# ChenJiahao031008/EAO-Fusion

Hardware: AMD Instinct MI355X
Metric: ORB kpts/s (640x480, 1k feat) + local-BA residuals/s (20 KF x 3k pts) (higher is better)
Workload: dtype u8; 1 GPU; ORBextractor FAST+rBRIEF, 640x480, 8-level pyramid, nFeatures 1000, batch=64 synthetic frames per GPU (BASELINE configs[1]); parallelism=frames sharded per GPU, no data-path collective

## Files before the change

### eao_fusion_amd/csrc/orb_host.hip

```cpp
#include "orb_internal.h"

using namespace eao::orb;

namespace eao {
namespace orb {

eao_status build_geometry(eao_orb* h, int W, int H) {
    const eao_orb_cfg& c = h->cfg;
    Geom& g = h->geom;
    std::memset(&g, 0, sizeof(g));
    g.nlevels = c.nlevels; g.W = W; g.H = H;
    g.iniTh = c.ini_th_fast; g.minTh = c.min_th_fast;
    for (int i = 0; i < 16; i++) g.umax[i] = h->umax[i];
    h->cells.clear();
    int off = 0, kpBase = 0, candBase = 0, tileBase = 0, maxCell = 0, scanCap = 0, maxList = 0, maxSw = 0, maxSh = 0;
    for (int l = 0; l < c.nlevels; l++) {
        LevelGeom& L = g.L[l];
        const float s = h->invScale[l];
        L.w = cv_round((float)W * s);
        L.h = cv_round((float)H * s);
        EAO_REQUIRE(L.w < 4096 && L.h < 4096, "level %d is %dx%d: coordinates are packed in 12 bits", l, L.w, L.h);
        const int maxBX = L.w - kEdge + 3, maxBY = L.h - kEdge + 3;
        const float width = (float)(maxBX - kMinBorder), height = (float)(maxBY - kMinBorder);
        const int nCols = (int)(width / (float)refc::FAST_CELL), nRows = (int)(height / (float)refc::FAST_CELL);
// ... 348 lines not shown
    const int nl = cfg->nlevels;
    const double scaleFactor = cfg->scale_factor;
    h->scale.resize(nl); h->sigma2.resize(nl); h->invScale.resize(nl); h->invSigma2.resize(nl); h->quota.resize(nl);
    h->scale[0] = 1.0f; h->sigma2[0] = 1.0f;
    for (int i = 1; i < nl; i++) {
        h->scale[i] = (float)(h->scale[i - 1] * scaleFactor);
        h->sigma2[i] = h->scale[i] * h->scale[i];
    }
    for (int i = 0; i < nl; i++) {
        h->invScale[i] = 1.0f / h->scale[i];
        h->invSigma2[i] = 1.0f / h->sigma2[i];
    }
    const float factor = (float)(1.0f / scaleFactor);
    float desired = cfg->nfeatures * (1 - factor) / (1 - (float)std::pow((double)factor, (double)nl));
    int sum = 0;
    for (int l = 0; l < nl - 1; l++) {
        h->quota[l] = cv_round(desired);
        sum += h->quota[l];
        desired *= factor;
    }
    h->quota[nl - 1] = std::max(cfg->nfeatures - sum, 0);
    {
        const int vmax = (int)std::floor(15 * std::sqrt(2.f) / 2 + 1), vmin = (int)std::ceil(15 * std::sqrt(2.f) / 2);
        for (int v = 0; v <= vmax; ++v) h->umax[v] = cv_round(std::sqrt(225.0 - v * v));
        for (int v = 15, v0 = 0; v >= vmin; --v) {
            while (h->umax[v0] == h->umax[v0 + 1]) ++v0;
            h->umax[v] = v0;
            ++v0;
        }
    }
    {
        const int expect[16] = {15, 15, 15, 15, 14, 14, 14, 13, 13, 12, 11, 10, 9, 8, 6, 3};
        for (int i = 0; i < 16; i++)
            if (h->umax[i] != expect[i]) { delete h; eao::set_error("umax table mismatch"); return EAO_ERR_INTERNAL; }
    }
    *out = h;
    return EAO_OK;
}

void eao_orb_destroy(eao_orb* h) {
    if (!h) return;
    for (hipEvent_t e : h->evs) if (e) (void)hipEventDestroy(e);
    if (h->stream) { (void)hipStreamSynchronize(h->stream); (void)hipStreamDestroy(h->stream); }
    for (hipStream_t q : {h->spacer, h->side}) if (q) { (void)hipStreamSynchronize(q); (void)hipStreamDestroy(q); }
    for (hipEvent_t e : {h->evFork, h->evFast0, h->evMid, h->evJoin}) if (e) (void)hipEventDestroy(e);
    if (h->pinOut) (void)hipHostFree(h->pinOut);
    if (h->pinUp) (void)hipHostFree(h->pinUp);
    if (h->pinPyr) (void)hipHostFree(h->pinPyr);
    stream_release(h);
    if (h->evStart) (void)hipEventDestroy(h->evStart);
    if (h->evLast) (void)hipEventDestroy(h->evLast);
    delete h;
}

eao_status eao_orb_tables(const eao_orb* h, float* scale, float* inv_scale, float* sigma2, float* inv_sigma2, int32_t* fpl) {
    EAO_REQUIRE(h, "null handle");
    for (int i = 0; i < h->cfg.nlevels; i++) {
        if (scale) scale[i] = h->scale[i];
        if (inv_scale) inv_scale[i] = h->invScale[i];
        if (sigma2) sigma2[i] = h->sigma2[i];
        if (inv_sigma2) inv_sigma2[i] = h->invSigma2[i];
        if (fpl) fpl[i] = h->quota[i];
    }
    return EAO_OK;
}

eao_status eao_orb_max_keypoints(eao_orb* h, int32_t width, int32_t height, int32_t* cap) {
    EAO_REQUIRE(h && cap, "null argument");
    eao_status st = ensure(h, width, height, 0);
    if (st) return st;
    *cap = h->geom.totalKpCap;
    return EAO_OK;
}

eao_status eao_orb_extract_batch_device(eao_orb* h, const uint8_t* d_img, int32_t width, int32_t height, int32_t stride,
                                        int64_t frame_stride, int32_t batch, eao_keypoint* d_kps, uint8_t* d_desc, int32_t cap,
                                        int32_t* d_n, void* stream) {
    EAO_REQUIRE(h && d_img && d_kps && d_desc && d_n, "null argument");
    EAO_REQUIRE(width > 0 && height > 0 && stride >= width && batch >= 1, "bad image geometry");
    eao_status st = ensure(h, width, height, batch, (hipStream_t)stream);
    if (st) return st;
    if (cap < h->geom.totalKpCap) {
        eao::set_error("cap %d < eao_orb_max_keypoints %d", cap, h->geom.totalKpCap);
        return EAO_ERR_CAPACITY;
    }
    return enqueue(h, d_img, stride, frame_stride, batch, d_kps, d_desc, cap, d_n, (hipStream_t)stream);
}

eao_status eao_orb_extract_batch(eao_orb* h, const uint8_t* img, int32_t width, int32_t height, int32_t stride, int64_t frame_stride,
                                 int32_t batch, eao_keypoint* kps, uint8_t* desc, int32_t cap, int32_t* n) {
    EAO_REQUIRE(h && n, "null argument");
    if (!img || width <= 0 || height <= 0) {
        for (int f = 0; f < std::max(batch, 0); f++) n[f] = 0;
        return EAO_OK;
    }
    EAO_REQUIRE(kps && desc && stride >= width && batch >= 1, "bad argument");
    eao_status st = ensure(h, width, height, batch);
    if (st) return st;
    const Geom& g = h->geom;
    if (cap < g.totalKpCap) {
        eao::set_error("cap %d < eao_orb_max_keypoints %d", cap, g.totalKpCap);
        return EAO_ERR_CAPACITY;
    }
    const size_t B = batch;
    if ((st = h->d_in.reserve(B * (size_t)g.L[0].pitch * height))) return st;
    if ((st = h->d_kps.reserve(B * (size_t)cap))) return st;
    if ((st = h->d_desc.reserve(B * (size_t)cap * 32))) return st;
    if ((st = h->d_nout.reserve(B))) return st;
    const long long fs0 = (long long)g.L[0].pitch * height;
    if ((st = upload_frames(h, img, width, height, stride, frame_stride, batch))) return st;
    const size_t outBytes = B * sizeof(int) + 64 + B * (size_t)cap * (sizeof(eao_keypoint) + 32);
    if (outBytes <= kPinnedOutMax) {
        if (h->pinOutCap < outBytes) {
            if (h->pinOut) (void)hipHostFree(h->pinOut);
            h->pinOut = nullptr; h->pinOutCap = 0;
            EAO_HIP(hipHostMalloc((void**)&h->pinOut, outBytes, hipHostMallocMapped));
            h->pinOutCap = outBytes;
        }
        unsigned char* dv = nullptr;
        EAO_HIP(hipHostGetDevicePointer((void**)&dv, h->pinOut, 0));
        const size_t offK = (B * sizeof(int) + 63) & ~(size_t)63, offD = offK + B * (size_t)cap * sizeof(eao_keypoint);
        st = enqueue(h, h->d_in.p, g.L[0].pitch, fs0, batch, (eao_keypoint*)(dv + offK), dv + offD, cap, (int*)dv, h->stream);
        if (st) return st;
        EAO_HIP(eao::wait_latency(h->stream));
        h->lastComplete = true;
        const int* hn = (const int*)h->pinOut;
        for (int f = 0; f < batch; f++) {
            const int nf = std::min(std::max(hn[f], 0), cap);
            n[f] = nf;
            std::memcpy(kps + (size_t)f * cap, h->pinOut + offK + (size_t)f * cap * sizeof(eao_keypoint), (size_t)nf * sizeof(eao_keypoint));
            std::memcpy(desc + (size_t)f * cap * 32, h->pinOut + offD + (size_t)f * cap * 32, (size_t)nf * 32);
        }
        return EAO_OK;
    }
    st = enqueue(h, h->d_in.p, g.L[0].pitch, fs0, batch, h->d_kps.p, h->d_desc.p, cap, h->d_nout.p, h->stream);
    if (st) return st;
    EAO_HIP(hipMemcpyAsync(n, h->d_nout.p, B * sizeof(int), hipMemcpyDeviceToHost, h->stream));
    EAO_HIP(hipMemcpyAsync(kps, h->d_kps.p, B * cap * sizeof(eao_keypoint), hipMemcpyDeviceToHost, h->stream));
    EAO_HIP(hipMemcpyAsync(desc, h->d_desc.p, B * (size_t)cap * 32, hipMemcpyDeviceToHost, h->stream));
    EAO_HIP(eao::wait_latency(h->stream));
    h->lastComplete = true;
    return EAO_OK;
}

eao_status eao_orb_extract(eao_orb* h, const uint8_t* img, int32_t width, int32_t height, int32_t stride, eao_keypoint* kps,
                           uint8_t* desc, int32_t cap, int32_t* n) {
    return eao_orb_extract_batch(h, img, width, height, stride, 0, 1, kps, desc, cap, n);
}

eao_status eao_orb_stream_create(eao_orb* h, int32_t width, int32_t height, int32_t batch, int32_t nslots) {
    EAO_REQUIRE(h && width > 0 && height > 0 && batch >= 1 && nslots >= 1 && nslots <= 8, "bad argument (1..8 slots)");
    eao_status st = ensure(h, width, height, batch);
    if (st) return st;
    stream_release(h);
    const Geom& g = h->geom;
    h->sW = width; h->sH = height; h->sB = batch; h->sCap = g.totalKpCap; h->sPitch = g.L[0].pitch;
    const size_t B = batch, cap = h->sCap;
    h->sInBytes = B * (size_t)h->sPitch * height;
    h->sOffK = eao::align256(B * sizeof(int));
    h->sOffD = eao::align256(h->sOffK + B * cap * sizeof(eao_keypoint));
    h->sOutBytes = (h->sOffD + B * cap * 32 + 15) & ~(size_t)15;
    EAO_HIP(eao::create_stream(&h->sUp, eao::StreamClass::Latency));
    EAO_HIP(eao::create_stream(&h->sRun, eao::StreamClass::Latency));
    EAO_HIP(eao::create_stream(&h->sDown, eao::StreamClass::Latency));
    h->slots.resize(nslots);
    for (eao_orb::StreamSlot& sl : h->slots) {
        EAO_HIP(hipHostMalloc((void**)&sl.pinIn, h->sInBytes, hipHostMallocDefault));
        EAO_HIP(hipHostMalloc((void**)&sl.pinOut, h->sOutBytes, hipHostMallocMapped));
        EAO_HIP(hipHostGetDevicePointer((void**)&sl.pinOutDev, sl.pinOut, 0));
        EAO_HIP(hipMalloc((void**)&sl.dIn, h->sInBytes));
        EAO_HIP(hipMalloc((void**)&sl.dOut, h->sOutBytes));
        EAO_HIP(hipEventCreateWithFlags(&sl.evIn, hipEventDisableTiming));
        EAO_HIP(hipEventCreateWithFlags(&sl.evOut, hipEventDisableTiming));
        EAO_HIP(hipEventCreateWithFlags(&sl.evDone, hipEventDisableTiming));
        std::memset(sl.pinOut, 0, h->sOutBytes);
    }
    return EAO_OK;
}

eao_status eao_orb_stream_slot(eao_orb* h, int32_t slot, eao_orb_slot* out) {
    EAO_REQUIRE(h && out && slot >= 0 && slot < (int)h->slots.size(), "no such slot (eao_orb_stream_create first)");
    const eao_orb::StreamSlot& sl = h->slots[slot];
    out->frames = sl.pinIn; out->stride = h->sPitch; out->frame_stride = (int64_t)h->sPitch * h->sH;
    out->n = (int32_t*)sl.pinOut; out->kps = (eao_keypoint*)(sl.pinOut + h->sOffK); out->desc = sl.pinOut + h->sOffD; out->cap = h->sCap;
    return EAO_OK;
}

eao_status eao_orb_stream_wait(eao_orb* h, int32_t slot) {
    EAO_REQUIRE(h && slot >= 0 && slot < (int)h->slots.size(), "no such slot (eao_orb_stream_create first)");
    eao_orb::StreamSlot& sl = h->slots[slot];
    EAO_REQUIRE(sl.submitted, "slot %d was not submitted", slot);
    EAO_HIP(hipEventSynchronize(sl.evOut));
    EAO_HIP(hipGetLastError());
    return EAO_OK;
}

eao_status eao_orb_level(eao_orb* h, int32_t frame, int32_t level, int32_t which, int32_t* w, int32_t* hgt, uint8_t* dst) {
    EAO_REQUIRE(h && h->geomValid && h->lastBatch > 0, "no extraction has run on this handle");
    EAO_REQUIRE(frame >= 0 && frame < h->lastBatch && level >= 0 && level < h->geom.nlevels, "frame/level out of range");
    const LevelGeom& L = h->geom.L[level];
    if (w) *w = L.w;
    if (hgt) *hgt = L.h;
    if (!dst) return EAO_OK;
    const uint8_t* src;
    int pitch;
    if (which == 0 && level == 0) {
        src = h->lastSrc.img0 + (long long)frame * h->lastSrc.fs0;
        pitch = h->lastSrc.pitch0;
    } else {
        src = (which ? h->d_blur.p : h->d_pyr.p) + (long long)frame * h->geom.pyrFrameBytes + L.off;
        pitch = L.pitch;
    }
    eao_status st = wait_last_extraction(h);
    if (st) return st;
    EAO_HIP(hipMemcpy2DAsync(dst, L.w, src, pitch, L.w, L.h, hipMemcpyDeviceToHost, h->stream));
    EAO_HIP(eao::wait_latency(h->stream));
    return EAO_OK;
}

eao_status eao_orb_pyramid(eao_orb* h, int32_t frame, int32_t border, eao_orb_level_view* levels) {
    EAO_REQUIRE(h && levels && h->geomValid && h->lastBatch > 0, "no extraction has run on this handle");
    EAO_REQUIRE(frame >= 0 && frame < h->lastBatch && border >= 0 && border <= 64, "frame / border out of range");
    if (!(h->lastComplete && h->pyrFrame == frame && h->pyrBorder == border)) {
        eao_status st = wait_last_extraction(h);
        if (!st) st = enqueue_pyramid_export(h, frame, border);
        if (st) return st;
        EAO_HIP(eao::wait_latency(h->stream));
        EAO_HIP(hipGetLastError());
    }
    for (int l = 0; l < h->geom.nlevels; l++) levels[l] = h->pyrViews[l];
    return EAO_OK;
}

eao_status eao_orb_set_keep_pyramid(eao_orb* h, int32_t border) {
    EAO_REQUIRE(h && border >= -1 && border <= 64, "border: -1 (off) .. 64");
    h->autoPyrBorder = border;
    return EAO_OK;
}

eao_status eao_orb_extract_ref(eao_orb* h, const uint8_t* img, int32_t width, int32_t height, int32_t stride, const eao_keypoint** kps,
                               const uint8_t** desc, int32_t* n) {
    EAO_REQUIRE(h && kps && desc && n, "null argument");
    *kps = nullptr; *desc = nullptr; *n = 0;
    if (!img || width <= 0 || height <= 0) return EAO_OK;
    EAO_REQUIRE(stride >= width, "bad argument");
    eao_status st = ensure(h, width, height, 1);
    if (st) return st;
    const Geom& g = h->geom;
    const int cap = g.totalKpCap;
    const size_t offK = 64, offD = offK + (size_t)cap * sizeof(eao_keypoint), outBytes = offD + (size_t)cap * 32;
    if (h->pinOutCap < outBytes) {
        if (h->pinOut) (void)hipHostFree(h->pinOut);
        h->pinOut = nullptr; h->pinOutCap = 0;
        EAO_HIP(hipHostMalloc((void**)&h->pinOut, outBytes, hipHostMallocMapped));
        h->pinOutCap = outBytes;
    }
    unsigned char* dv = nullptr;
    EAO_HIP(hipHostGetDevicePointer((void**)&dv, h->pinOut, 0));
    if ((st = h->d_in.reserve((size_t)g.L[0].pitch * height))) return st;
    const long long fs0 = (long long)g.L[0].pitch * height;
    if ((st = upload_frames(h, img, width, height, stride, 0, 1))) return st;
    st = enqueue(h, h->d_in.p, g.L[0].pitch, fs0, 1, (eao_keypoint*)(dv + offK), dv + offD, cap, (int*)dv, h->stream);
    if (st) return st;
    if (h->autoPyrBorder >= 0 && (st = enqueue_pyramid_export(h, 0, h->autoPyrBorder))) return st;
    EAO_HIP(eao::wait_latency(h->stream));
    h->lastComplete = true;
    *n = std::min(std::max(*(const int*)h->pinOut, 0), cap);
    *kps = (const eao_keypoint*)(h->pinOut + offK);
    *desc = h->pinOut + offD;
    return EAO_OK;
}

int32_t eao_orb_lanes(int32_t) { return 1; }

eao_status eao_orb_set_profiling(eao_orb* h, int32_t on) {
    EAO_REQUIRE(h, "null handle");
    h->profiling = on != 0;
    h->evUsed = 0;
    return EAO_OK;
}

eao_status eao_orb_last_timing(eao_orb* h, float ms[6]) {
    EAO_REQUIRE(h && ms && h->evUsed >= kProfEvents, "no profiled call since eao_orb_set_profiling(h, 1)");
    const size_t calls = h->evUsed / kProfEvents;
    EAO_HIP(hipEventSynchronize(h->evs[h->evUsed - kProfEvents + 8]));
    double acc[6] = {0, 0, 0, 0, 0, 0};
    for (size_t c = 0; c < calls; c++) {
        hipEvent_t* ev = &h->evs[c * kProfEvents];
        float t;
        EAO_HIP(hipEventElapsedTime(&t, ev[0], ev[1])); acc[0] += t;
        EAO_HIP(hipEventElapsedTime(&t, ev[9], ev[2])); acc[1] += t;
        EAO_HIP(hipEventElapsedTime(&t, ev[2], ev[3])); acc[2] += t;
        EAO_HIP(hipEventElapsedTime(&t, ev[6], ev[7])); acc[3] += t;
        EAO_HIP(hipEventElapsedTime(&t, ev[4], ev[5])); acc[4] += t;
        EAO_HIP(hipEventElapsedTime(&t, ev[0], ev[8])); acc[5] += t;
    }
    for (int i = 0; i < 6; i++) ms[i] = (float)(acc[i] / calls);
    h->evUsed = 0;
    if (h->d_dbg) {
        long long st[16 * kMaxLevels];
        EAO_HIP(hipMemcpy(st, h->d_dbg, sizeof(st), hipMemcpyDeviceToHost));
        for (int l = 0; l < h->geom.nlevels; l++) {
            const long long* o = st + 16 * l;
            fprintf(stderr, "[eao quadtree stamps] level %d: M %lld S %lld passes %lld | setup %lld | multi-scan %lld hist %lld order %lld growth %lld rank %lld newlist %lld rehome %lld tail %lld | final %lld cycles\n",
                    l, o[10], o[11], o[9], o[0], o[1], o[2], o[3], o[4], o[5], o[6], o[7], 0LL, o[8]);
        }
    }
    return EAO_OK;
}

}
```

### eao_fusion_amd/csrc/orb_internal.h

```cpp
#pragma once

#include <algorithm>
#include <atomic>
#include <cmath>
#include <cstdlib>
#include <cstring>
#include <vector>

#include "common.h"
#include "orb_blur_tables.h"
#include "orb_resize_tables.h"


namespace eao {
namespace orb {

constexpr int kMaxLevels = 16;
constexpr int kEdge = refc::EDGE_THRESHOLD;
constexpr int kMinBorder = kEdge - 3;
constexpr int kTile = 72;
constexpr int kTileStrideWide = 80;
constexpr int kMaxIni = 16;
constexpr size_t kPinnedOutMax = 1 << 20;
constexpr int kFastXcdRun = 0;

struct LevelGeom {
    int w, h, pitch, off;
    int cellBase, nCells;
    int quota;
    int nIni, boxH;
    float hX;
    int listCap;
    int kpBase;
    int candBase, candCap;
    int tileBase, tilesX;
    int mOk, mTileBase;
    int mTilesX, mBlocksY;
    int mXIdx, mYIdx;
    long long nodeOff;
    int scaledPatch;
    float scale;
};

struct Geom {
    int nlevels, W, H;
    int totalCells, cellCap;
    int totalKpCap, totalCandCap, totalTiles;
    int mTotalTiles, mFragOff;
    int pyrFrameBytes;
    int iniTh, minTh;
    int scanCap;
    int qtLdsCand, qtKeysOff;
    int qtNodesGlobal;
    long long qtNodeFrameBytes;
    int fastMaxTested, fastTileBytes, fastLdsBytes, fastStride;
    int umax[16];
    LevelGeom L[kMaxLevels];
};

struct CellDesc {
    short level, x0, y0, sw, sh, offX, offY, pad;
};

struct ImgSrc {
    const uint8_t* img0;
    int pitch0;
    long long fs0;
    uint8_t* pyr;
};

__device__ __forceinline__ const uint8_t* level_ptr(const Geom* g, const ImgSrc& s, int l, int f, int* pitch) {
    if (l == 0) {
        *pitch = s.pitch0;
        return s.img0 + (long long)f * s.fs0;
    }
    *pitch = g->L[l].pitch;
    return s.pyr + (long long)f * g->pyrFrameBytes + g->L[l].off;
}

constexpr int kPyrTW = 128, kPyrTH = 32;
constexpr int kPyrThreads = 256;
struct PyrLevel { int w, h, pitch, off; double invX, invY; int ldsOff, ldsW, ldsH; int coefXOff, coefYOff; };
struct PyrArgs {
    int nlevels, tilesX, tilesY, pyrFrameBytes;
    int coefOff;
    int coefCap;
    PyrLevel L[kMaxLevels];
    const int4* ranges;
    const int2* coefX;
    const int2* coefY;
};

constexpr int kQTSmall = 1024, kQTLarge = 256;
constexpr int kQtNodeInts = 2 + 2 + 2 + 4 + 4 + 5;

constexpr size_t kProfEvents = 10;


__host__ __device__ inline int pyr_src_ofs(int d, double inv, int sn) {
    float fr = (float)(((double)d + 0.5) * inv - 0.5);
    int o = (int)floorf(fr);
    return o < 0 ? 0 : (o > sn - 1 ? sn - 1 : o);
}
__host__ __device__ inline int pyr_first_at_least(int bound, double inv, int sn, int dn) {
    if (bound <= 0) return 0;
    int d = (int)((double)bound / inv);
    d = d < 0 ? 0 : (d > dn ? dn : d);
    while (d > 0 && pyr_src_ofs(d - 1, inv, sn) >= bound) d--;
    while (d < dn && pyr_src_ofs(d, inv, sn) < bound) d++;
    return d;
}

constexpr int kBlurRows = 16;
constexpr int kBlurSegW = 128;
constexpr int kBlurStripsPerWg = 8;
inline int cv_round(double v) { return (int)std::lrint(v); }

}
}

struct eao_orb {
    using Geom = eao::orb::Geom; using CellDesc = eao::orb::CellDesc; using PyrArgs = eao::orb::PyrArgs; using ImgSrc = eao::orb::ImgSrc;
    eao_orb_cfg cfg;
    std::vector<float> scale, invScale, sigma2, invSigma2;
    std::vector<int> quota;
    int umax[16];
    Geom geom;
    bool geomValid = false;
    int batchCap = 0;
    std::vector<CellDesc> cells;
    size_t quadLds = 0;
    eao::DevBuf<int4> d_pyrRanges;
    eao::DevBuf<int2> d_pyrCoef;
    PyrArgs pyr;
    size_t pyrLds = 0;
    bool pyrFused = false;
    hipStream_t stream = nullptr;
    hipStream_t side = nullptr;
    hipStream_t spacer = nullptr;
    bool evLastValid = false;
    hipStream_t lastStream = nullptr;
    hipEvent_t evLast = nullptr;
    bool everyCallEvent = false, evLastRecorded = false;
    hipEvent_t evStart = nullptr, evFork = nullptr, evJoin = nullptr, evFast0 = nullptr, evMid = nullptr;
    eao::DevBuf<Geom> d_geom;
    eao::DevBuf<CellDesc> d_cells;
    eao::DevBuf<uint8_t> d_pyr, d_blur, d_in;
    eao::DevBuf<uint8_t> d_blurTab;
    eao::DevBuf<uint8_t> d_resizeTab;
    eao::orb::ResizeMLevel resizeM[eao::orb::kMaxLevels] = {};
    size_t resizeMRowsOff = 0, resizeMStripsOff = 0;
    eao::DevBuf<unsigned> d_cellcand, d_cand, d_levelkps;
    eao::DevBuf<unsigned short> d_nodeof;
    eao::DevBuf<unsigned char> d_qtnodes;
    eao::DevBuf<int> d_cellcnt, d_levelcnt, d_candcnt, d_nout;
    eao::DevBuf<eao_keypoint> d_kps;
    unsigned char* pinOut = nullptr;
    size_t pinOutCap = 0;
    unsigned char* pinUp = nullptr;
    size_t pinUpCap = 0;
    eao::DevBuf<uint8_t> d_desc;
    eao::DevBuf<float> d_xyr;
    eao::DevBuf<unsigned char> d_stereo;
    unsigned char* pinPyr = nullptr;
    size_t pinPyrCap = 0;
    eao_orb_level_view pyrViews[eao::orb::kMaxLevels] = {};
    int pyrFrame = -1, pyrBorder = -1;
    int autoPyrBorder = -1;
    bool lastComplete = false;
    ImgSrc lastSrc{};
    int lastBatch = 0;
    bool profiling = false;
    long long* d_dbg = nullptr;
    std::vector<hipEvent_t> evs;
    size_t evUsed = 0;
    struct StreamSlot {
        unsigned char* pinIn = nullptr; unsigned char* pinOut = nullptr;
        unsigned char* pinOutDev = nullptr;
        unsigned char* dIn = nullptr; unsigned char* dOut = nullptr;
        hipEvent_t evIn = nullptr, evDone = nullptr, evOut = nullptr;
        int batch = 0;
        bool submitted = false;
    };
    std::vector<StreamSlot> slots;
    hipStream_t sUp = nullptr, sRun = nullptr, sDown = nullptr;
    int sW = 0, sH = 0, sB = 0, sCap = 0, sPitch = 0;
    size_t sInBytes = 0, sOutBytes = 0, sOffK = 0, sOffD = 0;
};

namespace eao {
namespace orb {
constexpr uintptr_t kNoCallerStream = ~(uintptr_t)0;
eao_status ensure(eao_orb* h, int W, int H, int batch, hipStream_t caller = (hipStream_t)kNoCallerStream);
eao_status order_behind_last_call(eao_orb* h, hipStream_t st);
void stream_release(eao_orb* h);
eao_status wait_last_extraction(eao_orb* h);
eao_status upload_frames(eao_orb* h, const uint8_t* img, int width, int height, int stride, long long frame_stride, int batch);
eao_status enqueue(eao_orb* h, const uint8_t* d_img, int pitch0, long long fs0, int batch, eao_keypoint* d_kps, uint8_t* d_desc, int cap, int* d_n, hipStream_t st);
eao_status enqueue_pyramid_export(eao_orb* h, int frame, int border);
void launch_resize_mfma(const eao_orb* h, hipStream_t str, const ImgSrc& s, int l, int batch, int frameAffinity);
void launch_quadtree(const eao_orb* h, hipStream_t str, int nb, int f0, int lFirst, int nLev);
eao_status quadtree_reserve_lds(size_t bytes);
}
}
```

### eao_fusion_amd/csrc/orb_quadtree.hip

```cpp
#include "orb_internal.h"

using namespace eao::orb;

namespace {

template <int kQT>
__device__ int block_excl_scan(int* a, int n, int* wtmp) {
    const int t = threadIdx.x, lane = t & 63, wv = t >> 6;
    const int per = (n + kQT - 1) / kQT;
    const int b = min(t * per, n), e = min(b + per, n);
    int ssum = 0;
    for (int i = b; i < e; i++) ssum += a[i];
    int v = ssum;
    v += __builtin_amdgcn_update_dpp(0, v, 0x111, 0xF, 0xF, true);
    v += __builtin_amdgcn_update_dpp(0, v, 0x112, 0xF, 0xF, true);
    v += __builtin_amdgcn_update_dpp(0, v, 0x114, 0xF, 0xF, true);
    v += __builtin_amdgcn_update_dpp(0, v, 0x118, 0xF, 0xF, true);
    v += __builtin_amdgcn_update_dpp(0, v, 0x142, 0xA, 0xF, true);
    v += __builtin_amdgcn_update_dpp(0, v, 0x143, 0xC, 0xF, true);
    __syncthreads();
    if (lane == 63) wtmp[wv] = v;
    __syncthreads();
    int woff = 0, total = 0;
#pragma unroll
    for (int w = 0; w < kQT / 64; w++) {
        const int x = wtmp[w];
        if (w < wv) woff += x;
        total += x;
    }
    int run = woff + v - ssum;
    for (int i = b; i < e; i++) {
        const int x = a[i];
        a[i] = run;
        run += x;
    }
    __syncthreads();
    return total;
}

__device__ __forceinline__ int wave_excl_scan(int* a, int n, int lane) {
    const int per = (n + 63) >> 6;
    const int b = min(lane * per, n), e = min(b + per, n);
    int ssum = 0;
    for (int i = b; i < e; i++) ssum += a[i];
    int v = ssum;
    v += __builtin_amdgcn_update_dpp(0, v, 0x111, 0xF, 0xF, true);
    v += __builtin_amdgcn_update_dpp(0, v, 0x112, 0xF, 0xF, true);
    v += __builtin_amdgcn_update_dpp(0, v, 0x114, 0xF, 0xF, true);
    v += __builtin_amdgcn_update_dpp(0, v, 0x118, 0xF, 0xF, true);
    v += __builtin_amdgcn_update_dpp(0, v, 0x142, 0xA, 0xF, true);
    v += __builtin_amdgcn_update_dpp(0, v, 0x143, 0xC, 0xF, true);
    const int total = __builtin_amdgcn_readlane(v, 63);
    int run = v - ssum;
    for (int i = b; i < e; i++) {
        const int x = a[i];
        a[i] = run;
        run += x;
    }
    eao::wave_sync();
    return total;
}

constexpr unsigned kQtLeaf = 0xFFFFFFFFu;
__device__ __forceinline__ unsigned box_mid(short4 bx) {
    return (unsigned)(bx.x + ((bx.z - bx.x + 1) >> 1)) | ((unsigned)(bx.y + ((bx.w - bx.y + 1) >> 1)) << 16);
}
__device__ __forceinline__ int quadrant_mid(unsigned key, unsigned mid) {
    const unsigned x = key & 0xFFF, y = (key >> 12) & 0xFFF;
    return (x < (mid & 0xFFFFu) ? 0 : 1) + (y < (mid >> 16) ? 0 : 2);
}
__device__ __forceinline__ int quadrant(unsigned key, short4 bx) {
    const int x = key & 0xFFF, y = (key >> 12) & 0xFFF;
    const int mx = bx.x + ((bx.z - bx.x + 1) >> 1);
    const int my = bx.y + ((bx.w - bx.y + 1) >> 1);
    return (x < mx ? 0 : 1) + (y < my ? 0 : 2);
}

struct QtArgs {
    const Geom* g; const unsigned* cellcand; const int* cellcnt; unsigned* levelkps; int* levelcnt; int f, l, M;
    long long* dbg;
    unsigned* candOut;
};

template <int kQT, class KeyPtr, class NofPtr>
__device__ __forceinline__ void quadtree_body(const QtArgs& A, unsigned char* smem, int* wtmp, int* shv, KeyPtr keys, NofPtr nof) {
    const Geom* __restrict__ g = A.g;
    int& sh_S = shv[0]; int& sh_phase = shv[1]; int& sh_done = shv[2]; int& sh_rstar = shv[3]; int& sh_nexp = shv[4];
    long long* dbg = A.dbg;
    __shared__ long long dacc[11];
    if (dbg && threadIdx.x == 0) { for (int i = 0; i < 10; i++) dacc[i] = 0; dacc[10] = clock64(); }
#define QSTAMP(i) do { if (dbg && threadIdx.x == 0) { const long long now_ = clock64(); dacc[i] += now_ - dacc[10]; dacc[10] = now_; } } while (0)
    const int t = threadIdx.x, lane = t & 63;
    const int l = A.l, f = A.f, M = A.M;
    const LevelGeom L = g->L[l];
    const int LC = L.listCap, N = L.quota;
    short4* box0 = reinterpret_cast<short4*>(smem);
    short4* box1 = box0 + LC;
    int* cnt0 = reinterpret_cast<int*>(box1 + LC);
    int* cnt1 = cnt0 + LC;
    int* crk0 = cnt1 + LC;
    int* crk1 = crk0 + LC;
    unsigned* mid0 = reinterpret_cast<unsigned*>(crk1 + LC);
    unsigned* mid1 = mid0 + LC;
    int* childcnt = reinterpret_cast<int*>(mid1 + LC);
    int* childpos = childcnt + 4 * LC;
    unsigned long long* rkey = reinterpret_cast<unsigned long long*>(childpos);
    int* newpos = childpos + 4 * LC;
    int* order = newpos + LC;
    int* vlist = order + LC;
    int* procRank = vlist + LC;
    int* scanB = procRank + LC;
    int* scanA = scanB + LC;

    const long long cslot = (long long)f * g->totalCells + L.cellBase;
    for (int c = t; c < L.nCells; c += kQT) {
        const int o = scanA[c], n = (c + 1 < L.nCells ? scanA[c + 1] : M) - o;
        const unsigned* srcc = A.cellcand + (cslot + c) * g->cellCap;
        for (int j0 = 0; j0 < n; j0 += 16) {
            unsigned v[16];
#pragma unroll
            for (int u = 0; u < 16; u++) v[u] = srcc[min(j0 + u, n - 1)];
#pragma unroll
            for (int u = 0; u < 16; u++)
                if (j0 + u < n) { keys[o + j0 + u] = v[u]; A.candOut[o + j0 + u] = v[u]; }
        }
    }
    __syncthreads();
    const int nIni = L.nIni;
    if (t < nIni) {
        box0[t] = make_short4((short)(int)(L.hX * (float)t), 0, (short)(int)(L.hX * (float)(t + 1)), (short)L.boxH);
        cnt0[t] = 0;
        crk0[t] = t;
    }
    __syncthreads();
    for (int k0 = 0; k0 < M; k0 += kQT) {
        const int k = k0 + t;
        int ini = -1;
        if (k < M) {
            ini = min((int)((float)(keys[k] & 0xFFF) / L.hX), nIni - 1);
            nof[k] = (unsigned short)ini;
        }
        for (int i = 0; i < nIni; i++) {
            const unsigned long long m = __ballot(ini == i);
            if (m && (t & 63) == 0) atomicAdd(&cnt0[i], __popcll(m));
        }
    }
    __syncthreads();
    if (t == 0) {
        int S = 0;
        for (int i = 0; i < nIni; i++) {
            newpos[i] = S;
            if (cnt0[i] > 0) { box0[S] = box0[i]; cnt0[S] = cnt0[i]; crk0[S] = S; mid0[S] = cnt0[i] > 1 ? box_mid(box0[i]) : kQtLeaf; S++; }
        }
        sh_S = S; sh_phase = 0; sh_done = 0;
    }
    __syncthreads();
    if (nIni > 1) {
        for (int k = t; k < M; k += kQT) nof[k] = (unsigned short)newpos[nof[k]];
        __syncthreads();
    }

    QSTAMP(0);
    int diters = 0;
    short4* box = box0; short4* nbox = box1;
    unsigned* mid = mid0; unsigned* nmid = mid1;
    int* cnt = cnt0; int* ncnt = cnt1;
    int* crk = crk0; int* ncrk = crk1;
#define QT_WAVE_FENCE() eao::wave_sync()
    const int wv = t >> 6;
    for (int iter = 0; iter < 64 && !sh_done; iter++) {
        const int S = sh_S, phase = sh_phase;
        for (int i = t; i < S; i += kQT) {
            procRank[i] = -1;
            childcnt[4 * i] = 0; childcnt[4 * i + 1] = 0; childcnt[4 * i + 2] = 0; childcnt[4 * i + 3] = 0;
        }
        if (t == 0) { sh_rstar = 0x7FFFFFFF; sh_nexp = 0; }
        __syncthreads();
        int nCand = 0;
        if (wv == 0) {
            for (int i = lane; i < S; i += 64) scanA[i] = cnt[i] > 1 ? 1 : 0;
            QT_WAVE_FENCE();
            nCand = wave_excl_scan(scanA, S, lane);
            for (int i = lane; i < S; i += 64)
                if (cnt[i] > 1) vlist[scanA[i]] = i;
            QT_WAVE_FENCE();
        }
        QSTAMP(1);
        for (int k0 = 0; k0 < M; k0 += 4 * kQT) {
            int nd[4], bin[4];
            unsigned ky[4], md[4];
#pragma unroll
            for (int u = 0; u < 4; u++) { const int k = k0 + u * kQT + t; nd[u] = k < M ? (int)nof[k] : -1; ky[u] = k < M ? keys[k] : 0u; }
#pragma unroll
            for (int u = 0; u < 4; u++) md[u] = nd[u] >= 0 ? mid[nd[u]] : kQtLeaf;
#pragma unroll
            for (int u = 0; u < 4; u++) bin[u] = md[u] != kQtLeaf ? 4 * nd[u] + quadrant_mid(ky[u], md[u]) : -1;
#pragma unroll
            for (int u = 0; u < 4; u++) {
                if (k0 + u * kQT >= M) break;
                const int prev = __builtin_amdgcn_update_dpp(-2, bin[u], 0x138, 0xF, 0xF, false);
                const bool head = bin[u] != prev;
                const unsigned long long hm = __ballot(head);
                if (head && bin[u] >= 0) {
                    const unsigned long long rest = lane == 63 ? 0ull : (hm >> (lane + 1));
                    const int run = rest ? __ffsll((long long)rest) : 64 - lane;
                    atomicAdd(&childcnt[bin[u]], run);
                }
            }
        }
        __syncthreads();
        QSTAMP(2);
        if (phase == 1) {
            if (wv == 0) {
                for (int j = lane; j < nCand; j += 64) { const int me = vlist[j]; rkey[j] = ((unsigned long long)(unsigned)cnt[me] << 32) | (unsigned)crk[me]; }
                if (lane == 0) sh_nexp = nCand;
            }
            __syncthreads();
            const int nC2 = sh_nexp;
            int sl = 1;
            while (2 * sl * nC2 <= kQT && sl < 16) sl *= 2;
            for (int j0 = 0; j0 < nC2; j0 += kQT / sl) {
                const int j = j0 + t / sl, part = t & (sl - 1);
                int r = 0;
                if (j < nC2) {
                    const unsigned long long mk = rkey[j];
#pragma unroll 8
                    for (int u = part; u < nC2; u += sl) r += rkey[u] > mk;
                }
                for (int d = sl >> 1; d >= 1; d >>= 1) r += __shfl_xor(r, d);
                if (j < nC2 && part == 0) order[r] = vlist[j];
            }
            __syncthreads();
            if (t == 0) sh_nexp = 0;
        }
        QSTAMP(3);
        if (wv == 0) {
            if (phase == 0) {
                for (int j = lane; j < nCand; j += 64) order[j] = vlist[j];
                QT_WAVE_FENCE();
            }
            for (int r = lane; r < nCand; r += 64) {
                const int i = order[r];
                scanA[r] = (childcnt[4 * i] > 0) + (childcnt[4 * i + 1] > 0) + (childcnt[4 * i + 2] > 0) + (childcnt[4 * i + 3] > 0);
            }
            QT_WAVE_FENCE();
            wave_excl_scan(scanA, nCand, lane);
            int rstar = 0x7FFFFFFF;
            if (phase == 1) {
                for (int r = lane; r < nCand; r += 64) {
                    const int i = order[r];
                    const int ne = (childcnt[4 * i] > 0) + (childcnt[4 * i + 1] > 0) + (childcnt[4 * i + 2] > 0) + (childcnt[4 * i + 3] > 0);
                    if (S + scanA[r] + ne - (r + 1) >= N) rstar = min(rstar, r);
                }
                for (int d = 32; d >= 1; d >>= 1) rstar = min(rstar, __shfl_xor(rstar, d));
            }
            QSTAMP(4);
            const int nProc = (phase == 1 && rstar != 0x7FFFFFFF) ? rstar + 1 : nCand;
            int totalChildren = 0;
            if (nProc > 0) {
                const int i = order[nProc - 1];
                totalChildren = scanA[nProc - 1] + (childcnt[4 * i] > 0) + (childcnt[4 * i + 1] > 0) + (childcnt[4 * i + 2] > 0) + (childcnt[4 * i + 3] > 0);
            }
            for (int r = lane; r < nProc; r += 64) procRank[order[r]] = r;
            QT_WAVE_FENCE();
            for (int i = lane; i < S; i += 64) scanB[i] = procRank[i] < 0 ? 1 : 0;
            QT_WAVE_FENCE();
            wave_excl_scan(scanB, S, lane);
            QSTAMP(5);
            int myexp = 0;
            for (int i = lane; i < S; i += 64) {
                const int r = procRank[i];
                if (r < 0) {
                    const int p = totalChildren + scanB[i];
                    nbox[p] = box[i]; ncnt[p] = cnt[i]; ncrk[p] = crk[i]; nmid[p] = mid[i];
                    childpos[4 * i] = p; childpos[4 * i + 1] = p; childpos[4 * i + 2] = p; childpos[4 * i + 3] = p;
                } else {
                    const short4 b = box[i];
                    const short mx = (short)(b.x + ((b.z - b.x + 1) >> 1)), my = (short)(b.y + ((b.w - b.y + 1) >> 1));
                    const int ne = (childcnt[4 * i] > 0) + (childcnt[4 * i + 1] > 0) + (childcnt[4 * i + 2] > 0) + (childcnt[4 * i + 3] > 0);
                    int p = totalChildren - (scanA[r] + ne);
                    for (int q = 3; q >= 0; q--) {
                        const int c = childcnt[4 * i + q];
                        if (c > 0) {
                            short4 nb;
                            nb.x = (q & 1) ? mx : b.x; nb.z = (q & 1) ? b.z : mx;
                            nb.y = (q & 2) ? my : b.y; nb.w = (q & 2) ? b.w : my;
                            nbox[p] = nb; ncnt[p] = c; ncrk[p] = 4 * r + q; nmid[p] = c > 1 ? box_mid(nb) : kQtLeaf;
                            childpos[4 * i + q] = p;
                            p++;
                            myexp += c > 1;
                        }
                    }
                }
            }
            for (int d = 32; d >= 1; d >>= 1) myexp += __shfl_xor(myexp, d);
            if (lane == 0) {
                const int S2 = totalChildren + S - nProc;
                sh_S = S2;
                if (S2 >= N || S2 == S) sh_done = 1;
                else if (phase == 0 && S2 + 3 * myexp > N) sh_phase = 1;
            }
        }
        __syncthreads();
        QSTAMP(6);
        for (int k = t; k < M; k += kQT) {
            const int nd = nof[k];
            nof[k] = (unsigned short)childpos[4 * nd + quadrant_mid(keys[k], mid[nd])];
        }
        __syncthreads();
        QSTAMP(7);
        diters++;
        short4* tb = box; box = nbox; nbox = tb;
        unsigned* tm = mid; mid = nmid; nmid = tm;
        int* ti = cnt; cnt = ncnt; ncnt = ti;
        ti = crk; crk = ncrk; ncrk = ti;
    }
#undef QT_WAVE_FENCE
    const int S = sh_S;
    unsigned* best = reinterpret_cast<unsigned*>(scanB);
    for (int i = t; i < S; i += kQT) best[i] = 0;
    __syncthreads();
    for (int k = t; k < M; k += kQT) atomicMax(&best[nof[k]], ((keys[k] >> 24) << 20) | (0xFFFFFu - (unsigned)k));
    __syncthreads();
    unsigned* out = A.levelkps + (long long)f * g->totalKpCap + L.kpBase;
    for (int i = t; i < S; i += kQT) {
        const unsigned k = 0xFFFFFu - (best[i] & 0xFFFFFu);
        out[i] = keys[k];
    }
    if (t == 0) A.levelcnt[f * g->nlevels + l] = S;
    QSTAMP(8);
    if (dbg && t == 0 && A.dbg) {
        long long* o = dbg + 16 * l;
        for (int i = 0; i < 9; i++) o[i] = dacc[i];
        o[9] = diters; o[10] = M; o[11] = S;
    }
#undef QSTAMP
}

template <int kQT>
__device__ __noinline__ void quadtree_global(const Geom* __restrict__ g, const unsigned* cellcand, const int* cellcnt, unsigned* cand, unsigned short* nodeof,
                                             unsigned* levelkps, int* levelcnt, int* candcnt, int f, int l, unsigned char* base, long long* dbg, int* wtmp, int* shv) {
    const int t = threadIdx.x;
    const LevelGeom L = g->L[l];
    int* scanA = reinterpret_cast<int*>(base + (size_t)L.listCap * (2 * sizeof(short4) + sizeof(int) * kQtNodeInts));
    const long long cslot = (long long)f * g->totalCells + L.cellBase;
    for (int i = t; i < L.nCells; i += kQT) scanA[i] = cellcnt[cslot + i];
    __syncthreads();
    const int M = block_excl_scan<kQT>(scanA, L.nCells, wtmp);
    if (t == 0) candcnt[f * g->nlevels + l] = M;
    if (M == 0) {
        if (t == 0) levelcnt[f * g->nlevels + l] = 0;
        return;
    }
    QtArgs A = {g, cellcand, cellcnt, levelkps, levelcnt, f, l, M, dbg, cand + (long long)f * g->totalCandCap + L.candBase};
    quadtree_body<kQT>(A, base, wtmp, shv, cand + (long long)f * g->totalCandCap + L.candBase, nodeof + (long long)f * g->totalCandCap + L.candBase);
}

template <int kQT>
__global__ __launch_bounds__(kQT, kQT == 256 ? 4 : 1) void k_quadtree(const Geom* __restrict__ g, const unsigned* __restrict__ cellcand,
                                                  const int* __restrict__ cellcnt, unsigned* __restrict__ cand,
                                                  unsigned short* __restrict__ nodeof, unsigned* __restrict__ levelkps,
                                                  int* __restrict__ levelcnt, int* __restrict__ candcnt, int f0, long long* dbg, int l0,
                                                  unsigned char* __restrict__ qtnodes) {
    extern __shared__ __align__(16) unsigned char smem[];
    __shared__ int wtmp[kQT / 64];
    __shared__ int shv[8];
    const int t = threadIdx.x;
    const int l = blockIdx.y + l0, f = blockIdx.x + f0;
    const LevelGeom L = g->L[l];
    if (g->qtNodesGlobal) {
        quadtree_global<kQT>(g, cellcand, cellcnt, cand, nodeof, levelkps, levelcnt, candcnt, f, l, qtnodes + (long long)f * g->qtNodeFrameBytes + L.nodeOff,
                        (dbg && f == f0) ? dbg : nullptr, wtmp, shv);
        return;
    }
    int* scanA = reinterpret_cast<int*>(smem + (size_t)L.listCap * (2 * sizeof(short4) + sizeof(int) * kQtNodeInts));
    const long long cslot = (long long)f * g->totalCells + L.cellBase;
    for (int i = t; i < L.nCells; i += kQT) scanA[i] = cellcnt[cslot + i];
    __syncthreads();
    const int M = block_excl_scan<kQT>(scanA, L.nCells, wtmp);
    if (t == 0) candcnt[f * g->nlevels + l] = M;
    if (M == 0) {
        if (t == 0) levelcnt[f * g->nlevels + l] = 0;
        return;
    }
    QtArgs A = {g, cellcand, cellcnt, levelkps, levelcnt, f, l, M, (dbg && f == f0) ? dbg : nullptr, cand + (long long)f * g->totalCandCap + L.candBase};
    if (M <= g->qtLdsCand) {
        unsigned* keysL = reinterpret_cast<unsigned*>(smem + g->qtKeysOff);
        quadtree_body<kQT>(A, smem, wtmp, shv, keysL, reinterpret_cast<unsigned short*>(keysL + g->qtLdsCand));
    } else {
        quadtree_body<kQT>(A, smem, wtmp, shv, cand + (long long)f * g->totalCandCap + L.candBase, nodeof + (long long)f * g->totalCandCap + L.candBase);
    }
}

}

void eao::orb::launch_quadtree(const eao_orb* h, hipStream_t str, int nb, int f0, int lFirst, int nLev) {
    if (nb < 36) hipLaunchKernelGGL(k_quadtree<kQTSmall>, dim3(nb, nLev), dim3(kQTSmall), h->quadLds, str, h->d_geom.p, h->d_cellcand.p, h->d_cellcnt.p, h->d_cand.p,
                       h->d_nodeof.p, h->d_levelkps.p, h->d_levelcnt.p, h->d_candcnt.p, f0, h->d_dbg, lFirst, h->d_qtnodes.p);
    else hipLaunchKernelGGL(k_quadtree<kQTLarge>, dim3(nb, nLev), dim3(kQTLarge), h->quadLds, str, h->d_geom.p, h->d_cellcand.p, h->d_cellcnt.p, h->d_cand.p,
                       h->d_nodeof.p, h->d_levelkps.p, h->d_levelcnt.p, h->d_candcnt.p, f0, h->d_dbg, lFirst, h->d_qtnodes.p);
}

eao_status eao::orb::quadtree_reserve_lds(size_t bytes) {
    static std::atomic<int> cur{0};
    int have = cur.load();
    while ((int)bytes > have) {
        EAO_HIP(hipFuncSetAttribute((const void*)k_quadtree<kQTSmall>, hipFuncAttributeMaxDynamicSharedMemorySize, (int)bytes));
        EAO_HIP(hipFuncSetAttribute((const void*)k_quadtree<kQTLarge>, hipFuncAttributeMaxDynamicSharedMemorySize, (int)bytes));
        if (cur.compare_exchange_weak(have, (int)bytes)) break;
    }
    return EAO_OK;
}
```

Measured before the change: 282.9 million kpts/s.

## Fuse quadtree rehome pass with next-iteration child histogram and double-buffer counts

```diff
diff --git a/eao_fusion_amd/csrc/orb_host.hip b/eao_fusion_amd/csrc/orb_host.hip
--- a/eao_fusion_amd/csrc/orb_host.hip
+++ b/eao_fusion_amd/csrc/orb_host.hip
@@ -674,7 +674,7 @@
         EAO_HIP(hipMemcpy(st, h->d_dbg, sizeof(st), hipMemcpyDeviceToHost));
         for (int l = 0; l < h->geom.nlevels; l++) {
             const long long* o = st + 16 * l;
-            fprintf(stderr, "[eao quadtree stamps] level %d: M %lld S %lld passes %lld | setup %lld | multi-scan %lld hist %lld order %lld growth %lld rank %lld newlist %lld rehome %lld tail %lld | final %lld cycles\n",
+            fprintf(stderr, "[eao quadtree stamps] level %d: M %lld S %lld passes %lld | setup %lld | multi-scan %lld hist(initial) %lld order %lld growth %lld rank %lld newlist %lld rehome+hist %lld tail %lld | final %lld cycles\n",
                     l, o[10], o[11], o[9], o[0], o[1], o[2], o[3], o[4], o[5], o[6], o[7], 0LL, o[8]);
         }
     }
diff --git a/eao_fusion_amd/csrc/orb_internal.h b/eao_fusion_amd/csrc/orb_internal.h
--- a/eao_fusion_amd/csrc/orb_internal.h
+++ b/eao_fusion_amd/csrc/orb_internal.h
@@ -92,7 +92,7 @@
 };
 
 constexpr int kQTSmall = 1024, kQTLarge = 256;
-constexpr int kQtNodeInts = 2 + 2 + 2 + 4 + 4 + 5;
+constexpr int kQtNodeInts = 2 + 2 + 2 + 8 + 4 + 4;
 
 constexpr size_t kProfEvents = 10;
 
diff --git a/eao_fusion_amd/csrc/orb_quadtree.hip b/eao_fusion_amd/csrc/orb_quadtree.hip
--- a/eao_fusion_amd/csrc/orb_quadtree.hip
+++ b/eao_fusion_amd/csrc/orb_quadtree.hip
@@ -74,6 +74,56 @@
     const int mx = bx.x + ((bx.z - bx.x + 1) >> 1);
     const int my = bx.y + ((bx.w - bx.y + 1) >> 1);
     return (x < mx ? 0 : 1) + (y < my ? 0 : 2);
+}
+
+template <int kQT, int kNR, bool kFull, class KeyPtr, class NofPtr>
+__device__ __forceinline__ void rehome_and_count_rows(KeyPtr keys, NofPtr nof, int M, int k0, const unsigned* mid, const int* childpos, const unsigned* nmid, int* cc, bool count) {
+    const int t = threadIdx.x, lane = t & 63;
+    int nd[kNR], bin[kNR];
+    unsigned ky[kNR], md[kNR];
+    bool in[kNR];
+#pragma unroll
+    for (int u = 0; u < kNR; u++) {
+        const int k = k0 + u * kQT + t;
+        in[u] = kFull || u < kNR - 1 || k < M;
+        const int kk = in[u] ? k : M - 1;
+        const int n = (int)nof[kk];
+        ky[u] = keys[kk];
+        nd[u] = in[u] ? n : 0;
+    }
+#pragma unroll
+    for (int u = 0; u < kNR; u++) md[u] = mid[nd[u]];
+#pragma unroll
+    for (int u = 0; u < kNR; u++) { const int n = childpos[4 * nd[u] + quadrant_mid(ky[u], md[u])]; nd[u] = in[u] ? n : 0; }
+#pragma unroll
+    for (int u = 0; u < kNR; u++) { const int k = k0 + u * kQT + t; if (in[u]) nof[k] = (unsigned short)nd[u]; }
+    if (!count) return;
+#pragma unroll
+    for (int u = 0; u < kNR; u++) md[u] = nmid[nd[u]];
+#pragma unroll
+    for (int u = 0; u < kNR; u++) bin[u] = in[u] && md[u] != kQtLeaf ? 4 * nd[u] + quadrant_mid(ky[u], md[u]) : -1;
+#pragma unroll
+    for (int u = 0; u < kNR; u++) {
+        const int prev = __builtin_amdgcn_update_dpp(-2, bin[u], 0x138, 0xF, 0xF, false);
+        const bool head = bin[u] != prev;
+        const unsigned long long hm = __ballot(head);
+        if (head && bin[u] >= 0) {
+            const unsigned long long rest = lane == 63 ? 0ull : (hm >> (lane + 1));
+            const int run = rest ? __ffsll((long long)rest) : 64 - lane;
+            atomicAdd(&cc[bin[u]], run);
+        }
+    }
+}
+
+template <int kQT, class KeyPtr, class NofPtr>
+__device__ __forceinline__ void rehome_and_count(KeyPtr keys, NofPtr nof, int M, const unsigned* mid, const int* childpos, const unsigned* nmid, int* cc, bool count) {
+    int k0 = 0;
+    for (; k0 + 4 * kQT <= M; k0 += 4 * kQT) rehome_and_count_rows<kQT, 4, true>(keys, nof, M, k0, mid, childpos, nmid, cc, count);
+    const int rest = M - k0;
+    if (rest > 3 * kQT) rehome_and_count_rows<kQT, 4, false>(keys, nof, M, k0, mid, childpos, nmid, cc, count);
+    else if (rest > 2 * kQT) rehome_and_count_rows<kQT, 3, false>(keys, nof, M, k0, mid, childpos, nmid, cc, count);
+    else if (rest > kQT) rehome_and_count_rows<kQT, 2, false>(keys, nof, M, k0, mid, childpos, nmid, cc, count);
+    else if (rest > 0) rehome_and_count_rows<kQT, 1, false>(keys, nof, M, k0, mid, childpos, nmid, cc, count);
 }
 
 struct QtArgs {
@@ -102,27 +152,48 @@
     int* crk1 = crk0 + LC;
     unsigned* mid0 = reinterpret_cast<unsigned*>(crk1 + LC);
     unsigned* mid1 = mid0 + LC;
-    int* childcnt = reinterpret_cast<int*>(mid1 + LC);
-    int* childpos = childcnt + 4 * LC;
+    int* childcnt0 = reinterpret_cast<int*>(mid1 + LC);
+    int* childcnt1 = childcnt0 + 4 * LC;
+    int* childpos = childcnt1 + 4 * LC;
     unsigned long long* rkey = reinterpret_cast<unsigned long long*>(childpos);
-    int* newpos = childpos + 4 * LC;
-    int* order = newpos + LC;
+    int* order = childpos + 4 * LC;
     int* vlist = order + LC;
     int* procRank = vlist + LC;
     int* scanB = procRank + LC;
     int* scanA = scanB + LC;
 
     const long long cslot = (long long)f * g->totalCells + L.cellBase;
-    for (int c = t; c < L.nCells; c += kQT) {
-        const int o = scanA[c], n = (c + 1 < L.nCells ? scanA[c + 1] : M) - o;
-        const unsigned* srcc = A.cellcand + (cslot + c) * g->cellCap;
-        for (int j0 = 0; j0 < n; j0 += 16) {
-            unsigned v[16];
-#pragma unroll
-            for (int u = 0; u < 16; u++) v[u] = srcc[min(j0 + u, n - 1)];
-#pragma unroll
-            for (int u = 0; u < 16; u++)
-                if (j0 + u < n) { keys[o + j0 + u] = v[u]; A.candOut[o + j0 + u] = v[u]; }
+    {
+        constexpr int kGL = 16, kGC = 8, kGroups = kQT / kGL;
+        const int grp = t / kGL, gl = t % kGL;
+        const int cellCap = g->cellCap;
+        for (int c0 = 0; c0 < L.nCells; c0 += kGroups * kGC) {
+            int o[kGC], n[kGC];
+            unsigned va[kGC], vb[kGC];
+#pragma unroll
+            for (int u = 0; u < kGC; u++) {
+                const int c = c0 + u * kGroups + grp, cc = min(c, L.nCells - 1);
+                o[u] = scanA[cc];
+                const int e = cc + 1 < L.nCells ? scanA[cc + 1] : M;
+                n[u] = c < L.nCells ? e - o[u] : 0;
+            }
+#pragma unroll
+            for (int u = 0; u < kGC; u++) {
+                const unsigned* srcc = A.cellcand + (cslot + min(c0 + u * kGroups + grp, L.nCells - 1)) * cellCap;
+                va[u] = srcc[min(gl, cellCap - 1)];
+                vb[u] = srcc[min(gl + kGL, cellCap - 1)];
+            }
+#pragma unroll
+            for (int u = 0; u < kGC; u++) {
+                if (gl < n[u]) { keys[o[u] + gl] = va[u]; A.candOut[o[u] + gl] = va[u]; }
+                if (gl + kGL < n[u]) { keys[o[u] + gl + kGL] = vb[u]; A.candOut[o[u] + gl + kGL] = vb[u]; }
+            }
+#pragma unroll
+            for (int u = 0; u < kGC; u++) {
+                if (n[u] <= 2 * kGL) continue;
+                const unsigned* srcc = A.cellcand + (cslot + c0 + u * kGroups + grp) * cellCap;
+                for (int j = gl + 2 * kGL; j < n[u]; j += kGL) { const unsigned v = srcc[j]; keys[o[u] + j] = v; A.candOut[o[u] + j] = v; }
+            }
         }
     }
     __syncthreads();
@@ -131,8 +202,15 @@
         box0[t] = make_short4((short)(int)(L.hX * (float)t), 0, (short)(int)(L.hX * (float)(t + 1)), (short)L.boxH);
         cnt0[t] = 0;
         crk0[t] = t;
-    }
-    __syncthreads();
+        mid1[t] = kQtLeaf;
+        procRank[t] = -1;
+        childcnt0[4 * t] = 0; childcnt0[4 * t + 1] = 0; childcnt0[4 * t + 2] = 0; childcnt0[4 * t + 3] = 0;
+    }
+    __syncthreads();
+    if (nIni == 1) {
+        for (int k = t; k < M; k += kQT) nof[k] = 0;
+        if (t == 0) cnt0[0] = M;
+    } else
     for (int k0 = 0; k0 < M; k0 += kQT) {
         const int k = k0 + t;
         int ini = -1;
@@ -149,33 +227,27 @@
     if (t == 0) {
         int S = 0;
         for (int i = 0; i < nIni; i++) {
-            newpos[i] = S;
+            childpos[4 * i] = S;
             if (cnt0[i] > 0) { box0[S] = box0[i]; cnt0[S] = cnt0[i]; crk0[S] = S; mid0[S] = cnt0[i] > 1 ? box_mid(box0[i]) : kQtLeaf; S++; }
         }
-        sh_S = S; sh_phase = 0; sh_done = 0;
-    }
-    __syncthreads();
-    if (nIni > 1) {
-        for (int k = t; k < M; k += kQT) nof[k] = (unsigned short)newpos[nof[k]];
-        __syncthreads();
-    }
-
+        sh_S = S; sh_phase = 0; sh_done = 0; sh_rstar = 0x7FFFFFFF; sh_nexp = 0;
+    }
+    __syncthreads();
     QSTAMP(0);
+    int S = sh_S, phase = sh_phase, done = 0;
+    rehome_and_count<kQT>(keys, nof, M, mid1, childpos, mid0, childcnt0, true);
+    __syncthreads();
+    QSTAMP(2);
+
     int diters = 0;
     short4* box = box0; short4* nbox = box1;
     unsigned* mid = mid0; unsigned* nmid = mid1;
     int* cnt = cnt0; int* ncnt = cnt1;
     int* crk = crk0; int* ncrk = crk1;
+    int* childcnt = childcnt0; int* nchildcnt = childcnt1;
 #define QT_WAVE_FENCE() eao::wave_sync()
     const int wv = t >> 6;
-    for (int iter = 0; iter < 64 && !sh_done; iter++) {
-        const int S = sh_S, phase = sh_phase;
-        for (int i = t; i < S; i += kQT) {
-            procRank[i] = -1;
-            childcnt[4 * i] = 0; childcnt[4 * i + 1] = 0; childcnt[4 * i + 2] = 0; childcnt[4 * i + 3] = 0;
-        }
-        if (t == 0) { sh_rstar = 0x7FFFFFFF; sh_nexp = 0; }
-        __syncthreads();
+    for (int iter = 0; iter < 64 && !done; iter++) {
         int nCand = 0;
         if (wv == 0) {
             for (int i = lane; i < S; i += 64) scanA[i] = cnt[i] > 1 ? 1 : 0;
@@ -186,30 +258,6 @@
             QT_WAVE_FENCE();
         }
         QSTAMP(1);
-        for (int k0 = 0; k0 < M; k0 += 4 * kQT) {
-            int nd[4], bin[4];
-            unsigned ky[4], md[4];
-#pragma unroll
-            for (int u = 0; u < 4; u++) { const int k = k0 + u * kQT + t; nd[u] = k < M ? (int)nof[k] : -1; ky[u] = k < M ? keys[k] : 0u; }
-#pragma unroll
-            for (int u = 0; u < 4; u++) md[u] = nd[u] >= 0 ? mid[nd[u]] : kQtLeaf;
-#pragma unroll
-            for (int u = 0; u < 4; u++) bin[u] = md[u] != kQtLeaf ? 4 * nd[u] + quadrant_mid(ky[u], md[u]) : -1;
-#pragma unroll
-            for (int u = 0; u < 4; u++) {
-                if (k0 + u * kQT >= M) break;
-                const int prev = __builtin_amdgcn_update_dpp(-2, bin[u], 0x138, 0xF, 0xF, false);
-                const bool head = bin[u] != prev;
-                const unsigned long long hm = __ballot(head);
-                if (head && bin[u] >= 0) {
-                    const unsigned long long rest = lane == 63 ? 0ull : (hm >> (lane + 1));
-                    const int run = rest ? __ffsll((long long)rest) : 64 - lane;
-                    atomicAdd(&childcnt[bin[u]], run);
-                }
-            }
-        }
-        __syncthreads();
-        QSTAMP(2);
         if (phase == 1) {
             if (wv == 0) {
                 for (int j = lane; j < nCand; j += 64) { const int me = vlist[j]; rkey[j] = ((unsigned long long)(unsigned)cnt[me] << 32) | (unsigned)crk[me]; }
@@ -300,13 +348,15 @@
                 if (S2 >= N || S2 == S) sh_done = 1;
                 else if (phase == 0 && S2 + 3 * myexp > N) sh_phase = 1;
             }
+        } else {
+            const int nz = 4 * min(LC, 4 * S);
+            for (int i = t - 64; i < nz; i += kQT - 64) nchildcnt[i] = 0;
         }
         __syncthreads();
         QSTAMP(6);
-        for (int k = t; k < M; k += kQT) {
-            const int nd = nof[k];
-            nof[k] = (unsigned short)childpos[4 * nd + quadrant_mid(keys[k], mid[nd])];
-        }
+        S = sh_S; phase = sh_phase; done = sh_done;
+        for (int i = t; i < S; i += kQT) procRank[i] = -1;
+        rehome_and_count<kQT>(keys, nof, M, mid, childpos, nmid, nchildcnt, !done);
         __syncthreads();
         QSTAMP(7);
         diters++;
@@ -314,9 +364,9 @@
         unsigned* tm = mid; mid = nmid; nmid = tm;
         int* ti = cnt; cnt = ncnt; ncnt = ti;
         ti = crk; crk = ncrk; ncrk = ti;
+        ti = childcnt; childcnt = nchildcnt; nchildcnt = ti;
     }
 #undef QT_WAVE_FENCE
-    const int S = sh_S;
     unsigned* best = reinterpret_cast<unsigned*>(scanB);
     for (int i = t; i < S; i += kQT) best[i] = 0;
     __syncthreads();
```

Result: faster. 293.8 million kpts/s (median of 6 runs) (+3.9%).
